# google/dynamic-video-depth

Hardware: AMD Instinct MI355X
Metric: train iters/s (depth+sceneflow step) at 384x672, 48 pairs; warp+loss HBM GB/s (higher is better)
Workload: dtype f32 (storage and accumulation fp32; conv / MLP contractions on v_mfma_f32_32x32x16_f16: every fp32 operand, scaled by a power of two from its tensor's max, is split into two fp16 terms (22 bits) and a product is three partial products; <= 4e-6 of max|y| against float64, the bound the 3-term bf16 / 6

## Files before the change

### dynamic-video-depth_amd/dvd_hip/csrc/xconv.hip

```cpp
#include <type_traits>

#include "dvd_split.h"
#include "xconv_tile.h"

namespace dvd {

typedef float f32x16 __attribute__((ext_vector_type(16)));
typedef float f32x2 __attribute__((ext_vector_type(2)));
typedef unsigned u32x4 __attribute__((ext_vector_type(4)));

#ifndef DVD_XCONV_ROLL
#define DVD_XCONV_ROLL 1
#endif
#ifndef DVD_XCONV_SPARE
#define DVD_XCONV_SPARE 0
#endif
#ifndef DVD_XCONV_DIRECT_BATCH
#define DVD_XCONV_DIRECT_BATCH 4
#endif
constexpr int kXHeader = 16;

__device__ __forceinline__ float xconv_weight(const float* __restrict__ w, int co_g, int idx, const float* __restrict__ sc_gamma,
                                              const float* __restrict__ sc_var, float sc_eps) {
  float val = w[idx];
// ... 134 lines not shown
      for (int k = 0; k < 4; ++k) m = fmaxf(fmaxf(m, fmaxf(fabsf(v[k].x), fabsf(v[k].y))), fmaxf(fabsf(v[k].z), fabsf(v[k].w)));
      if (it.var) m *= fabsf((it.gamma ? it.gamma[row] : 1.0f) / sqrtf(it.var[row] + it.eps));
      mall = fmaxf(mall, m);
    }
  } else {
    for (int row = blockIdx.x * kWamaxWaves + wave; row < it.rows; row += gridDim.x * kWamaxWaves) {
      const float* wr = it.w + (size_t)row * it.row_len;
      float m = 0.0f;
      for (int i = lane; i < it.row_len; i += 64) m = fmaxf(m, fabsf(wr[i]));
      if (it.var) m *= fabsf((it.gamma ? it.gamma[row] : 1.0f) / sqrtf(it.var[row] + it.eps));
      mall = fmaxf(mall, m);
    }
  }
  block_partial_max<kWamaxWaves>(mall, reinterpret_cast<float*>(it.packed));
}

__global__ __launch_bounds__(256) void xconv_pack_many_kernel(const XPackDev* __restrict__ table, int n) {
  int lo = 0, hi = n - 1;
  while (lo < hi) {
    const int mid = (lo + hi + 1) >> 1;
    if (table[mid].block0 <= blockIdx.x) lo = mid; else hi = mid - 1;
  }
  const XPackDev it = table[lo];
  xconv_pack_block(it.w, it.packed, it.co, it.ci, it.T, it.transposed, it.mtiles, it.nkc, it.G, it.gamma, it.var, it.eps,
                   kManyPartials, blockIdx.x - it.block0);
}

struct XArgs {
  const void* __restrict__ x;
  const uint4* __restrict__ wp;
  const float* __restrict__ bias;
  const void* __restrict__ res;
  const void* __restrict__ mask_src;
  const float* __restrict__ bn_gamma;
  const float* __restrict__ bn_beta;
  const float* __restrict__ bn_mean;
  const float* __restrict__ bn_var;
  float bn_eps;
  const float* __restrict__ x_amax;
  float* y_amax;
  void* __restrict__ y;
  int N, Cin, Cout, H, W;
  int G, mbpg, mtiles;
  int KS, pad, T;
  int TR, TC, P, ntr, ntc, NV;
  int PQ;
  int nkc, npos, nfi;
  int relu_in, relu_out, res_relu;
  int vec_out;
  int Hi, Wi, S2, ZI;
};

constexpr int kXFitOne = 11;
template <int TM, int TN, int WM, int WN, int FIT, bool FAST, bool B1 = false, bool IN16 = false, bool OUT16 = false>
__global__ __launch_bounds__(64 * WM * WN, B1 ? 3 : 2) void xconv_kernel(const XArgs a) {
  static_assert(!IN16 || FAST, "fp16 activations exist on the buffer-addressed main loop only");
  using TX = std::conditional_t<IN16, _Float16, float>;
  using TY = std::conditional_t<OUT16, _Float16, float>;
  using RawT = std::conditional_t<IN16, unsigned short, float>;
  constexpr int BT = IN16 ? 1 : 2;
  constexpr int XB = IN16 ? 2 : 4;
  constexpr int NT = 64 * WM * WN;
  constexpr bool kDirect = FIT == 0;
  constexpr bool kOne = FIT == kXFitOne;
  constexpr int FI = (kDirect || kOne) ? 1 : FIT;
  constexpr int MT = WM * TM;
  constexpr int AU = MT * 2 * 64;
  constexpr int AI = (AU + NT - 1) / NT;
  constexpr int AS = AI * NT;
  extern __shared__ __attribute__((aligned(16))) u32x4 smem[];
  u32x4* sA = smem;
  u32x4* sB = smem + 2 * AS;
  const int tid = threadIdx.x, lane = tid & 63, wave = tid >> 6;
  const int wm = wave / WN, wn = wave - wm * WN;
  const int tr = blockIdx.x / a.ntc, tc = blockIdx.x - tr * a.ntc;
  const int r0 = tr * a.TR, c0 = tc * a.TC;
  const int grp = blockIdx.y / a.mbpg;
  const int mt0 = (blockIdx.y - grp * a.mbpg) * MT;
  const int n = blockIdx.z;
  const size_t plane = (size_t)a.H * a.W;
  const size_t planeI = (size_t)a.Hi * a.Wi;
  const TX* xn = static_cast<const TX*>(a.x) + ((size_t)n * a.G + grp) * a.Cin * planeI;
  const int npos = a.npos, P = a.P, T = a.T, KS = a.KS;
  const int nkt = a.nkc * T;

  auto locate = [&](int p, bool live, int& go, bool& ok, int& lp) {
    if (a.S2) {
      const int PI = 2 * a.TC + 1;
      const int rr = p / PI, cc = p - rr * PI;
      const int row = 2 * r0 - 1 + rr, col = 2 * c0 - 1 + cc;
      ok = live && row >= 0 && row < a.Hi && col >= 0 && col < a.Wi;
      go = ok ? (row * a.Wi + col) : 0;
      lp = ((rr & 1) * 2 + (cc & 1)) * a.S2 + (rr >> 1) * P + (cc >> 1);
      return;
    }
    const int rr = p / P, cc = p - rr * P;
    const int row = r0 - a.pad + rr, col = c0 - a.pad + cc;
    ok = live && row >= 0 && row < a.H && col >= 0 && col < a.W;
    if (a.ZI) {
      ok = ok && !((row | col) & 1);
      go = ok ? ((row >> 1) * a.Wi + (col >> 1)) : 0;
    } else {
      go = ok ? (row * a.W + col) : 0;
    }
    lp = p;
  };
  auto tapoff = [&](int ky, int kx) { return xconv_tapoff(ky, kx, P, a.S2); };
  int goff[FI], lidx[FI], cig8[FI];
  bool gok[FI];
#pragma unroll
  for (int it = 0; it < FI; ++it) {
    const int item = it * NT + tid;
    const int cig = item >= a.NV ? 1 : 0;
    const int p = item - cig * a.NV;
    const bool live = item < 2 * a.NV;
    int lp;
    locate(p, live, goff[it], gok[it], lp);
    lidx[it] = live ? (cig * npos + lp) : (npos - 1);
    cig8[it] = live ? cig * 8 : 0;
  }
  const int planeB = (int)planeI * XB;
  const float sx = IN16 ? 1.0f : pow2_scale(a.x_amax[0]);
  const float sw = pow2_scale(reinterpret_cast<const float*>(a.wp)[0]);
  int voff[FI];
#pragma unroll
// ... 162 lines not shown
        }
      }
      uint4 h, l;
      split8_f16(v, sx, h, l);
      dst[li] = (u32x4){h.x, h.y, h.z, h.w};
      dst[2 * npos + li] = (u32x4){l.x, l.y, l.z, l.w};
    }
  };

  const u32x4* asrc[AI];
#pragma unroll
  for (int i = 0; i < AI; ++i) {
    const int j = i * NT + tid;
    const int jj = j < AU ? j : 0;
    const int mtl = jj / 128, rem = jj - mtl * 128;
    asrc[i] = reinterpret_cast<const u32x4*>(a.wp) + kXHeader + ((size_t)(grp * a.mtiles + mt0 + mtl) * nkt) * 128 + rem;
  }
  const u32x4* abase = reinterpret_cast<const u32x4*>(a.wp) + kXHeader + ((size_t)(grp * a.mtiles + mt0) * nkt) * 128;
  const __amdgpu_buffer_rsrc_t srdA = __builtin_amdgcn_make_buffer_rsrc(
      uniform_ptr(const_cast<u32x4*>(abase)), 0, FAST ? MT * nkt * 128 * 16 : 0, 0x00020000);
  int aoff[AI];
#pragma unroll
  for (int i = 0; i < AI; ++i) {
    const int j = i * NT + tid;
    const int jj = j < AU ? j : 0;
    const int mtl = jj / 128, rem = jj - mtl * 128;
    aoff[i] = (mtl * nkt * 128 + rem) * 16;
  }
  struct ARegs {
    u32x4 v[AI];
  };
  auto load_a = [&](ARegs& r, int kt) {
    if (FAST) {
#pragma unroll
      for (int i = 0; i < AI; ++i)
        r.v[i] = __builtin_bit_cast(u32x4, __builtin_amdgcn_raw_buffer_load_b128(srdA, aoff[i], kt * 2048, 0));
      return;
    }
#pragma unroll
    for (int i = 0; i < AI; ++i) r.v[i] = asrc[i][(size_t)kt * 128];
  };
  auto write_a = [&](const ARegs& r, int buf) {
#pragma unroll
    for (int i = 0; i < AI; ++i) sA[buf * AS + i * NT + tid] = r.v[i];
  };

  f32x16 acc[TM][TN];
#pragma unroll
  for (int tm = 0; tm < TM; ++tm)
#pragma unroll
    for (int tn = 0; tn < TN; ++tn) acc[tm][tn] = (f32x16){0, 0, 0, 0, 0, 0, 0, 0, 0, 0, 0, 0, 0, 0, 0, 0};

  auto qpos = [&](int tn) { return (wn * TN + tn) * 32 + (lane & 31); };
  constexpr bool kPackCells = TM >= 4 && !kOne;
  constexpr int QP = kPackCells ? (TN + 1) / 2 : TN;
  int qbp[QP];
#pragma unroll
  for (int h = 0; h < QP; ++h) {
    if constexpr (kPackCells) {
      const int c0 = xconv_cell(qpos(2 * h), a.PQ, P, a.TR);
      const int c1 = 2 * h + 1 >= TN ? 0 : xconv_cell(qpos(2 * h + 1), a.PQ, P, a.TR);
      qbp[h] = c0 | (c1 << 16);
    } else {
      qbp[h] = kOne ? 0 : xconv_cell(qpos(h), a.PQ, P, a.TR);
    }
  }
  auto cells = [&](int (&qb)[TN]) {
    if constexpr (kOne) {
#pragma unroll
      for (int tn = 0; tn < TN; ++tn) qb[tn] = qpos(tn);
    } else if constexpr (!kPackCells) {
#pragma unroll
      for (int tn = 0; tn < TN; ++tn) qb[tn] = qbp[tn];
    } else {
#pragma unroll
      for (int h = 0; h < QP; ++h) {
        int pk = qbp[h];
        asm volatile("" : "+v"(pk));
        qb[2 * h] = pk & 0xffff;
        if (2 * h + 1 < TN) qb[2 * h + 1] = (int)((unsigned)pk >> 16);
      }
    }
  };
  const int bl = (lane >> 5) * npos;
  const int al = (wm * TM) * 128 + lane;

  struct Frag {
    f16x8 a[TM][2], b[TN][BT];
  };
  auto read_frags = [&](Frag& f, int abuf, int kc, int off) {
    const u32x4* Ac = sA + abuf * AS + al;
    const u32x4* Bc = sB + (B1 ? 0 : (kc & 1) * 2 * BT * npos) + bl + off;
    int qb[TN];
    cells(qb);
#pragma unroll
    for (int tm = 0; tm < TM; ++tm)
#pragma unroll
      for (int s = 0; s < 2; ++s) f.a[tm][s] = __builtin_bit_cast(f16x8, Ac[(tm * 2 + s) * 64]);
#pragma unroll
    for (int tn = 0; tn < TN; ++tn)
#pragma unroll
      for (int s = 0; s < BT; ++s) f.b[tn][s] = __builtin_bit_cast(f16x8, Bc[s * 2 * npos + qb[tn]]);
  };
  auto mfmas = [&](const Frag& f) {
#define DVD_XTERM(SA, SB)                                                                             \
  _Pragma("unroll") for (int tm = 0; tm < TM; ++tm) _Pragma("unroll") for (int tn = 0; tn < TN; ++tn) \
      acc[tm][tn] = __builtin_amdgcn_mfma_f32_32x32x16_f16(f.a[tm][SA], f.b[tn][SB], acc[tm][tn], 0, 0, 0);
    DVD_XTERM(1, 0)
    if constexpr (!IN16) { DVD_XTERM(0, 1) }
    DVD_XTERM(0, 0)
#undef DVD_XTERM
  };

  constexpr bool kSingleA = TM >= 4;
  constexpr bool kRoll = kSingleA && !B1 && (DVD_XCONV_ROLL != 0);
  ARegs ra, rb;
  if (kRoll) {
    load_a(ra, 0);
    if (!kDirect) load_raw(0);
    write_a(ra, 0);
    load_a(ra, nkt > 1 ? 1 : 0);
    if (kDirect) {
      stage_direct(0, 0);
      if (T == 1 && a.nkc > 1) stage_direct(1, 1);
    } else {
      split_write(0, 0);
      load_raw(a.nkc > 1 ? 1 : 0);
      if (T == 1) {
        if (a.nkc > 1) split_write(1, 1);
        load_raw(a.nkc > 2 ? 2 : 0);
      }
    }
    write_a(ra, 1);
    __syncthreads();
    f16x8 fa[TM][2], fb[2][TN][BT];
    {
      const u32x4* Ac = sA + al;
      const u32x4* Bc = sB + bl;
      int qb[TN];
      cells(qb);
#pragma unroll
      for (int tm = 0; tm < TM; ++tm)
#pragma unroll
        for (int t = 0; t < 2; ++t) fa[tm][t] = __builtin_bit_cast(f16x8, Ac[(tm * 2 + t) * 64]);
#pragma unroll
      for (int tn = 0; tn < TN; ++tn)
#pragma unroll
        for (int t = 0; t < BT; ++t) fb[0][tn][t] = __builtin_bit_cast(f16x8, Bc[t * 2 * npos + qb[tn]]);
    }
    int nc = 0, ny = 0, nx = 0;
    auto advance = [&]() {
      if (++nx == KS) {
        nx = 0;
        if (++ny == KS) {
          ny = 0;
          ++nc;
        }
      }
    };
    advance();
    auto step_roll = [&](int kt, f16x8 (&bc)[TN][BT], f16x8 (&bn)[TN][BT]) {
      __syncthreads();
      load_a(ra, kt + 2 < nkt ? kt + 2 : kt);
      const u32x4* Ac = sA + ((kt + 1) & 1) * AS + al;
      const u32x4* Bc = sB + (nc & 1) * 2 * BT * npos + bl + tapoff(ny, nx);
      int qb[TN];
      cells(qb);
#pragma unroll
      for (int tn = 0; tn < TN; ++tn)
#pragma unroll
// ... 89 lines not shown
    split_write(0, 0);
    load_raw(a.nkc > 1 ? 1 : 0);
  }

  int kc = 0, ky = 0, kx = 0;
  auto step = [&](int kt, ARegs& rn) {
    __syncthreads();
    Frag f;
    read_frags(f, kt & 1, kc, tapoff(ky, kx));
    if (kSingleA) {
      load_a(rn, kt + 1 < nkt ? kt + 1 : kt);
      __builtin_amdgcn_sched_barrier(0);
    }
    mfmas(f);
    write_a(rn, (kt + 1) & 1);
    if (!kSingleA) load_a(rn, kt + 3 < nkt ? kt + 3 : kt);
    if (++kx == KS) {
      kx = 0;
      if (++ky == KS) {
        ky = 0;
        if (B1) __syncthreads();
        if (kDirect) {
          if (kc + 1 < a.nkc) stage_direct((kc + 1) & 1, kc + 1);
        } else {
#if DVD_XCONV_SPARE
          split_write((kc + 1) & 1, kc + 1);
          load_raw(kc + 2 < a.nkc ? kc + 2 : kc);
#else
          if (kc + 1 < a.nkc) split_write((kc + 1) & 1, kc + 1);
          if (kc + 2 < a.nkc) load_raw(kc + 2);
#endif
        }
        ++kc;
      }
    }
  };
  if (kSingleA) {
    for (int kt = 0; kt < nkt; ++kt) step(kt, ra);
  } else {
    for (int kt = 0; kt < nkt; kt += 2) {
      step(kt, rb);
      if (kt + 1 < nkt) step(kt + 1, ra);
    }
  }
  }

  const int TRv = (a.H - r0) < a.TR ? (a.H - r0) : a.TR;
  const int TCv = (a.W - c0) < a.TC ? (a.W - c0) : a.TC;
  const size_t ibase = ((size_t)n * a.G + grp) * a.Cout * plane;
  TY* __restrict__ yb = static_cast<TY*>(a.y) + ibase;
  const int iplane = (int)plane;
  const float unscale = 1.0f / (sx * sw);
  float ymax = 0.0f;
  if constexpr (kOne) {
    if (a.vec_out) {
      constexpr int PXL = OUT16 ? 8 : 4;
      constexpr int LPR = 64 / PXL;
      constexpr int RPI = 64 / LPR;
      constexpr int kTP = 68;
      __syncthreads();
      float* Tw = reinterpret_cast<float*>(smem) + wave * (32 * kTP);
      const int j = lane & 31, hh = lane >> 5;
      const int px = (lane % LPR) * PXL, rl = lane / LPR;
      const int q0 = wn * TN * 32;
      const bool pok = q0 + px < TCv;
      float my_sc[TM], my_sh[TM];
#pragma unroll
      for (int tm = 0; tm < TM; ++tm) {
        my_sc[tm] = 1.0f;
        my_sh[tm] = 0.0f;
        if (a.bn_var) {
          const int co = (mt0 + wm * TM + tm) * 32 + (lane & 31);
          const int cg = grp * a.Cout + (co < a.Cout ? co : a.Cout - 1);
          my_sc[tm] = (a.bn_gamma ? a.bn_gamma[cg] : 1.0f) / sqrtf(a.bn_var[cg] + a.bn_eps);
          my_sh[tm] = (a.bn_beta ? a.bn_beta[cg] : 0.0f) - a.bn_mean[cg] * my_sc[tm];
        }
      }
#pragma unroll
      for (int tm = 0; tm < TM; ++tm) {
#pragma unroll
        for (int tn = 0; tn < TN; ++tn)
#pragma unroll
          for (int r = 0; r < 16; ++r)
            Tw[((r & 3) + 8 * (r >> 2) + 4 * hh) * kTP + tn * 32 + j] = acc[tm][tn][r] * unscale;
        __builtin_amdgcn_wave_barrier();
#pragma unroll
        for (int i = 0; i < 32 / RPI; ++i) {
          const int cl = rl + RPI * i;
          const int co = (mt0 + wm * TM + tm) * 32 + cl;
          const bool ok = pok && co < a.Cout;
          float v[PXL];
#pragma unroll
          for (int e4 = 0; e4 < PXL; e4 += 4) {
            const float4 t = *reinterpret_cast<const float4*>(Tw + cl * kTP + px + e4);
            v[e4] = t.x; v[e4 + 1] = t.y; v[e4 + 2] = t.z; v[e4 + 3] = t.w;
          }
          const int cg = grp * a.Cout + (co < a.Cout ? co : a.Cout - 1);
          if (a.bias) {
            const float b = a.bias[cg];
#pragma unroll
            for (int e = 0; e < PXL; ++e) v[e] += b;
          }
          if (a.bn_var) {
            const float sc = __shfl(my_sc[tm], cl, 64), sh = __shfl(my_sh[tm], cl, 64);
#pragma unroll
            for (int e = 0; e < PXL; ++e) v[e] = __builtin_fmaf(v[e], sc, sh);
          }
          const int o = ok ? co * iplane + c0 + q0 + px : 0;
          auto load_run = [&](const void* base, float (&d)[PXL]) {
            const TY* __restrict__ p = static_cast<const TY*>(base) + ibase + o;
            if constexpr (OUT16) {
              const u32x4 t = *reinterpret_cast<const u32x4*>(p);
#pragma unroll
              for (int e = 0; e < 4; ++e) {
                const f16x2 h2 = __builtin_bit_cast(f16x2, (unsigned)t[e]);
                d[2 * e] = (float)h2[0];
                d[2 * e + 1] = (float)h2[1];
              }
            } else {
              const float4 t = *reinterpret_cast<const float4*>(p);
              d[0] = t.x; d[1] = t.y; d[2] = t.z; d[3] = t.w;
            }
          };
          if (a.res) {
            float rv[PXL];
            load_run(a.res, rv);
#pragma unroll
            for (int e = 0; e < PXL; ++e) v[e] += a.res_relu ? fmaxf(rv[e], 0.0f) : rv[e];
          }
          if (a.mask_src) {
            float mv[PXL];
            load_run(a.mask_src, mv);
#pragma unroll
            for (int e = 0; e < PXL; ++e) v[e] = mv[e] > 0.0f ? v[e] : 0.0f;
          }
          if (a.relu_out) {
#pragma unroll
// ... 53 lines not shown
          const int co = cob + (r & 3) + 8 * (r >> 2);
          v[r] += a.bias[grp * a.Cout + (co < a.Cout ? co : a.Cout - 1)];
        }
      }
      if (a.bn_var) {
#pragma unroll
        for (int r = 0; r < 16; ++r) {
          const int src = (r & 3) + 8 * (r >> 2) + 4 * (lane >> 5);
          v[r] = __builtin_fmaf(v[r], __shfl(my_sc[tm], src, 64), __shfl(my_sh[tm], src, 64));
        }
      }
      if (a.res) {
        const TY* __restrict__ rb = static_cast<const TY*>(a.res) + ibase;
        float rv[16];
#pragma unroll
        for (int r = 0; r < 16; ++r) {
          const int co = cob + (r & 3) + 8 * (r >> 2);
          rv[r] = (float)rb[(full || co < a.Cout) ? o0 + ((r & 3) + 8 * (r >> 2)) * iplane : pix];
        }
#pragma unroll
        for (int r = 0; r < 16; ++r) v[r] += a.res_relu ? fmaxf(rv[r], 0.0f) : rv[r];
      }
      if (a.mask_src) {
        const TY* __restrict__ mb = static_cast<const TY*>(a.mask_src) + ibase;
        float mv[16];
#pragma unroll
        for (int r = 0; r < 16; ++r) {
          const int co = cob + (r & 3) + 8 * (r >> 2);
          mv[r] = (float)mb[(full || co < a.Cout) ? o0 + ((r & 3) + 8 * (r >> 2)) * iplane : pix];
        }
#pragma unroll
        for (int r = 0; r < 16; ++r) v[r] = mv[r] > 0.0f ? v[r] : 0.0f;
      }
      if (a.relu_out) {
#pragma unroll
        for (int r = 0; r < 16; ++r) v[r] = fmaxf(v[r], 0.0f);
      }
#pragma unroll
      for (int r = 0; r < 16; ++r) {
        const int co = cob + (r & 3) + 8 * (r >> 2);
        if (pok && (full || co < a.Cout)) {
          yb[o0 + ((r & 3) + 8 * (r >> 2)) * iplane] = (TY)v[r];
          ymax = amax_acc(ymax, v[r]);
        }
      }
    }
  }
  if (a.y_amax) wave_amax_to(ymax, a.y_amax);
}

static int g_xcfg = 0;

template <int TM, int TN, int WM, int WN, bool FAST, bool B1 = false, bool IN16 = false, bool OUT16 = false>
static int launch_fi(const XArgs& a, int FI, dim3 grid, size_t lds, hipStream_t s) {
  auto go = [&](auto kern) -> int {
    DVD_HIP_OK(hipFuncSetAttribute(reinterpret_cast<const void*>(kern), hipFuncAttributeMaxDynamicSharedMemorySize, (int)lds));
    hipLaunchKernelGGL(kern, grid, dim3(64 * WM * WN), lds, s, a);
    DVD_LAUNCH_OK();
    return DVD_OK;
  };
  const double flops = 2.0 * a.N * (double)a.G * a.Cout * a.Cin * a.T * (double)a.H * a.W * (a.ZI ? 0.25 : 1.0);
  if constexpr (TM >= 4 && !B1 && FAST && DVD_XCONV_ROLL != 0) {
    if (a.T == 1 && FI == 1 && g_xcfg != 6) {
      flops_add(DVD_FLOP_XCONV_1X1_WIDE, flops);
      return go(xconv_kernel<TM, TN, WM, WN, kXFitOne, FAST, B1, IN16, OUT16>);
    }
  }
  flops_add(TM >= 4 ? DVD_FLOP_XCONV_WIDE : (WM == 2 ? DVD_FLOP_XCONV_128 : DVD_FLOP_XCONV_SMALL), flops);
  switch (FI) {
    case 1: return go(xconv_kernel<TM, TN, WM, WN, 1, FAST, B1, IN16, OUT16>);
    case 2: return go(xconv_kernel<TM, TN, WM, WN, 2, FAST, B1, IN16, OUT16>);
    case 3: return go(xconv_kernel<TM, TN, WM, WN, 3, FAST, B1, IN16, OUT16>);
    default: return go(xconv_kernel<TM, TN, WM, WN, 0, FAST, B1, IN16, OUT16>);
  }
}

static int xconv_mtiles(int M) {
  const int bm = M <= 32 ? 32 : (M <= 64 ? 64 : (M >= 256 ? 256 : 128));
  return (M + bm - 1) / bm * (bm / 32);
}

}

extern "C" {

size_t dvd_xconv_packed_bytes(int Cout, int Cin, int KS, int groups, int transposed) {
  if (Cout <= 0 || Cin <= 0 || KS <= 0 || !(KS & 1) || groups <= 0 || Cout % groups || Cin % groups) return 0;
  const int co = Cout / groups, ci = Cin / groups;
  const int M = transposed ? ci : co, K = transposed ? co : ci;
  return ((size_t)dvd::kXHeader + (size_t)groups * dvd::xconv_mtiles(M) * ((K + 15) / 16) * KS * KS * 2 * 64) * sizeof(uint4);
}

static int xconv_pack_impl(const float* w, void* packed, int Cout, int Cin, int KS, int groups, int transposed,
                           const float* gamma, const float* var, float eps, dvd_stream_t stream) {
  DVD_REQUIRE(w && packed, "xconv_pack: null pointer");
  DVD_REQUIRE(Cout > 0 && Cin > 0 && KS > 0 && (KS & 1) && KS <= 11 && groups > 0 && Cout % groups == 0 && Cin % groups == 0,
              "xconv_pack: bad shape Cout=%d Cin=%d KS=%d groups=%d", Cout, Cin, KS, groups);
  const int co = Cout / groups, ci = Cin / groups;
  const int M = transposed ? ci : co, K = transposed ? co : ci;
  const int mtiles = dvd::xconv_mtiles(M), nkc = (K + 15) / 16, T = KS * KS;
  const long long total = (long long)groups * mtiles * nkc * T * 64;
  dvd::bytes_add(DVD_BYTES_PACK, 8.0 * (double)Cout * ci * T + 16.0 * (double)total);
  const int row_len = ci * T;
  int npart;
  if (row_len % 4 == 0 && reinterpret_cast<uintptr_t>(w) % 16 == 0) {
    const int cpr = (row_len + 1023) / 1024;
    const long long nb = ((long long)Cout * cpr + dvd::kWamaxWaves - 1) / dvd::kWamaxWaves;
    npart = (int)(nb < dvd::kXPartials ? nb : dvd::kXPartials);
    hipLaunchKernelGGL(dvd::xconv_wamax4_kernel, dim3((unsigned)npart), dim3(64 * dvd::kWamaxWaves), 0, static_cast<hipStream_t>(stream), w,
                       static_cast<float*>(packed), Cout, row_len, cpr, gamma, var, eps);
    DVD_LAUNCH_OK();
  } else {
    npart = Cout < dvd::kXPartials ? Cout : dvd::kXPartials;
    hipLaunchKernelGGL(dvd::xconv_wamax_kernel, dim3((unsigned)npart), dim3(256), 0, static_cast<hipStream_t>(stream), w,
                       static_cast<float*>(packed), Cout, row_len, gamma, var, eps);
    DVD_LAUNCH_OK();
  }
  hipLaunchKernelGGL(dvd::xconv_pack_kernel, dim3((unsigned)((total + 255) / 256)), dim3(256), 0,
                     static_cast<hipStream_t>(stream), w, static_cast<uint4*>(packed), co, ci, T, transposed ? 1 : 0,
                     mtiles, nkc, groups, gamma, var, eps, npart);
  DVD_LAUNCH_OK();
  return DVD_OK;
}

int dvd_xconv_pack(const float* w, void* packed, int Cout, int Cin, int KS, int groups, int transposed, dvd_stream_t stream) {
  return xconv_pack_impl(w, packed, Cout, Cin, KS, groups, transposed, nullptr, nullptr, 0.0f, stream);
// ... 9 lines not shown

int dvd_xconv_pack_many(const dvd_xpack_item* items, int n, void* table, size_t table_bytes, int upload, dvd_stream_t stream) {
  DVD_REQUIRE(items && table && n > 0, "xconv_pack_many: bad arguments");
  DVD_REQUIRE(table_bytes >= dvd_xconv_pack_table_bytes(n), "xconv_pack_many: table %zu < %zu bytes", table_bytes,
              dvd_xconv_pack_table_bytes(n));
  std::vector<dvd::XPackDev> host((size_t)n);
  unsigned long long blocks = 0;
  double bytes = 0.0;
  for (int i = 0; i < n; ++i) {
    const dvd_xpack_item& q = items[i];
    DVD_REQUIRE(q.w && q.packed, "xconv_pack_many: item %d: null pointer", i);
    DVD_REQUIRE(q.Cout > 0 && q.Cin > 0 && q.KS > 0 && (q.KS & 1) && q.KS <= 11 && q.groups > 0 && q.Cout % q.groups == 0 &&
                    q.Cin % q.groups == 0,
                "xconv_pack_many: item %d: bad shape Cout=%d Cin=%d KS=%d groups=%d", i, q.Cout, q.Cin, q.KS, q.groups);
    DVD_REQUIRE(!q.gamma || q.var, "xconv_pack_many: item %d: BatchNorm scale without a variance", i);
    dvd::XPackDev& d = host[(size_t)i];
    d.w = q.w;
    d.packed = static_cast<uint4*>(q.packed);
    d.gamma = q.gamma;
    d.var = q.var;
    d.eps = q.eps;
    d.co = q.Cout / q.groups;
    d.ci = q.Cin / q.groups;
    d.T = q.KS * q.KS;
    d.transposed = q.transposed ? 1 : 0;
    const int M = d.transposed ? d.ci : d.co, K = d.transposed ? d.co : d.ci;
    d.mtiles = dvd::xconv_mtiles(M);
    d.nkc = (K + 15) / 16;
    d.G = q.groups;
    d.rows = q.Cout;
    d.row_len = d.ci * d.T;
    d.block0 = (unsigned)blocks;
    d.pad_ = 0;
    const long long total = (long long)d.G * d.mtiles * d.nkc * d.T * 64;
    blocks += (unsigned long long)((total + 255) / 256);
    bytes += 8.0 * (double)q.Cout * d.ci * d.T + 16.0 * (double)total;
  }
  DVD_REQUIRE(blocks < (1ull << 31), "xconv_pack_many: too many blocks");
  hipStream_t st = static_cast<hipStream_t>(stream);
  if (upload) {
    DVD_HIP_OK(hipMemcpyAsync(table, host.data(), (size_t)n * sizeof(dvd::XPackDev), hipMemcpyHostToDevice, st));
    DVD_HIP_OK(hipStreamSynchronize(st));
  }
  dvd::bytes_add(DVD_BYTES_PACK, bytes);
  const dvd::XPackDev* t = static_cast<const dvd::XPackDev*>(table);
  hipLaunchKernelGGL(dvd::xconv_wamax_many_kernel, dim3(dvd::kManyPartials, (unsigned)n), dim3(64 * dvd::kWamaxWaves), 0, st, t);
  DVD_LAUNCH_OK();
  hipLaunchKernelGGL(dvd::xconv_pack_many_kernel, dim3((unsigned)blocks), dim3(256), 0, st, t, n);
  DVD_LAUNCH_OK();
  return DVD_OK;
}

int dvd_xconv_select(int cfg) {
  DVD_REQUIRE(cfg >= 0 && cfg <= dvd::kXSelHalo, "xconv_select: cfg %d", cfg);
  dvd::g_xcfg = cfg;
  return DVD_OK;
}

static int xconv_fwd_impl(const void* x, const float* x_amax, const void* packed, const float* bias, const void* residual,
                          const void* mask_src, const dvd_bn_params* bn, void* y, float* y_amax, int N, int Cin_total,
                          int Cout_total, int H, int W, int KS, int groups, int flags, int in16, int out16, dvd_stream_t stream) {
  DVD_REQUIRE(x && packed && y, "xconv: null pointer");
  DVD_REQUIRE(in16 || x_amax, "xconv: the input's max|x| scalar is missing (dvd_amax, or the producer's y_amax)");
  DVD_REQUIRE(N > 0 && Cin_total > 0 && Cout_total > 0 && H > 0 && W > 0, "xconv: bad shape N=%d Cin=%d Cout=%d H=%d W=%d", N,
              Cin_total, Cout_total, H, W);
  DVD_REQUIRE(groups > 0 && Cin_total % groups == 0 && Cout_total % groups == 0, "xconv: %d groups do not divide the channels",
              groups);
  DVD_REQUIRE(KS > 0 && (KS & 1) && KS <= 11, "xconv: kernel size %d (odd sizes up to 11)", KS);
  DVD_REQUIRE(N <= 65535, "xconv: too many images for the grid");
  DVD_REQUIRE((long long)H * W * (long long)(Cin_total > Cout_total ? Cin_total : Cout_total) < (1ll << 31),
              "xconv: image too large for 32-bit offsets");
  DVD_REQUIRE(in16 || !out16, "xconv: fp32 input with fp16 output is not a configuration of this kernel");
  const int s2 = (flags >> 3) & 1, zi = (flags >> 4) & 1;
  DVD_REQUIRE(!(s2 && zi), "xconv: stride-2 forward and stride-2 backward-data are different launches");
  DVD_REQUIRE(!(s2 || zi) || KS == 3, "xconv: the strided forms exist for 3x3 kernels (got %d)", KS);
  const int Hq = (H + 1) / 2, Wq = (W + 1) / 2;
  const int Cin = Cin_total / groups, Cout = Cout_total / groups;
  dvd::XPlan plan;
  const bool planned = dvd::xconv_plan(Cin, Cout, H, W, KS, s2 != 0, in16 != 0, dvd::g_xcfg, plan);
  const bool fast = plan.fast;
  DVD_REQUIRE(fast || !in16, "xconv: fp16 activations need input channels in multiples of 16 (got %d per group)", Cin);
  DVD_REQUIRE(!(s2 || zi) || fast, "xconv: the strided forms need input channels in multiples of 16 (got %d per group)", Cin);
  DVD_REQUIRE(planned, "xconv: no %stile of a %dx%d image with a %dx%d kernel fits the LDS", s2 ? "stride-2 " : "", H, W, KS, KS);
  const dvd::XCfg& c = plan.c;
  const dvd::XTile& t = plan.t;
  const int Hh = plan.Hh, Ww = plan.Ww, S2 = plan.S2;
  dvd::XArgs a;
  a.x = x;
  a.wp = static_cast<const uint4*>(packed);
  a.bias = bias;
  a.res = residual;
  a.mask_src = mask_src;
  a.bn_gamma = bn ? bn->gamma : nullptr;
  a.bn_beta = bn ? bn->beta : nullptr;
  a.bn_mean = bn ? bn->mean : nullptr;
  a.bn_var = bn ? bn->var : nullptr;
  a.bn_eps = bn ? bn->eps : 0.0f;
  DVD_REQUIRE(!bn || (bn->mean && bn->var), "xconv: BatchNorm statistics missing");
  a.y = y;
  a.x_amax = x_amax;
  a.y_amax = y_amax;
  a.N = N; a.Cin = Cin; a.Cout = Cout; a.H = Hh; a.W = Ww;
  a.G = groups; a.mtiles = dvd::xconv_mtiles(Cout);
  a.KS = KS; a.pad = KS / 2; a.T = KS * KS;
  a.TR = t.TR; a.TC = t.TC; a.P = t.P; a.PQ = t.PQ; a.ntr = t.ntr; a.ntc = t.ntc; a.NV = t.NV;
  a.nkc = (Cin + 15) / 16; a.npos = t.npos; a.nfi = t.FI;
  a.Hi = s2 ? H : (zi ? Hq : Hh); a.Wi = s2 ? W : (zi ? Wq : Ww); a.S2 = S2; a.ZI = zi;
  a.relu_in = flags & 1; a.relu_out = (flags >> 1) & 1; a.res_relu = (flags >> 2) & 1;
  const int mblocks = plan.mblocks;
  a.mbpg = mblocks;
  DVD_REQUIRE((long long)mblocks * groups <= 65535, "xconv: too many channel blocks");
  const dim3 grid(t.ntr * t.ntc, mblocks * groups, N);
  auto al16 = [](const void* p) { return (reinterpret_cast<uintptr_t>(p) & 15) == 0; };
  a.vec_out = (KS == 1 && ((long long)H * W) % 8 == 0 && t.TC % 8 == 0 && al16(y) && al16(residual) && al16(mask_src) &&
               dvd::g_xcfg != 7) ? 1 : 0;
  size_t lds = t.lds;
  if (a.vec_out && lds < (size_t)c.NT() / 64 * 32 * 68 * 4) lds = (size_t)c.NT() / 64 * 32 * 68 * 4;
  hipStream_t s = static_cast<hipStream_t>(stream);
#define DVD_XGO(TM_, TN_, WM_, WN_)                                                                                      \
  do {                                                                                                                   \
    if (in16 && out16) return dvd::launch_fi<TM_, TN_, WM_, WN_, true, false, true, true>(a, t.FI, grid, lds, s);         \
    if (in16) return dvd::launch_fi<TM_, TN_, WM_, WN_, true, false, true, false>(a, t.FI, grid, lds, s);                 \
    return dvd::launch_fi<TM_, TN_, WM_, WN_, true>(a, t.FI, grid, lds, s);                                               \
  } while (0)
  if (fast) {
    if (c.TM == 4 && c.WN == 4) DVD_XGO(4, 2, 2, 4);
    if (c.TM == 4) DVD_XGO(4, 2, 2, 2);
    if (c.WM == 2 && c.b1) return dvd::launch_fi<2, 2, 2, 2, true, true>(a, t.FI, grid, lds, s);
    if (c.TM == 2 && c.WM == 1 && c.b1) return dvd::launch_fi<2, 2, 1, 4, true, true>(a, t.FI, grid, lds, s);
    if (c.TM == 1 && c.b1) return dvd::launch_fi<1, 2, 1, 4, true, true>(a, t.FI, grid, lds, s);
    if (c.WM == 2) DVD_XGO(2, 2, 2, 2);
    if (c.TM == 2) DVD_XGO(2, 2, 1, 4);
    DVD_XGO(1, 2, 1, 4);
  }
#undef DVD_XGO
  if (c.WM == 2) return dvd::launch_fi<2, 2, 2, 2, false>(a, t.FI, grid, lds, s);
  if (c.TM == 2) return dvd::launch_fi<2, 2, 1, 4, false>(a, t.FI, grid, lds, s);
  return dvd::launch_fi<1, 2, 1, 4, false>(a, t.FI, grid, lds, s);
}

int dvd_xconv_fwd(const float* x, const float* x_amax, const void* packed, const float* bias, const float* residual,
                  const float* mask_src, const dvd_bn_params* bn, float* y, float* y_amax, int N, int Cin_total, int Cout_total,
                  int H, int W, int KS, int groups, int flags, dvd_stream_t stream) {
  return xconv_fwd_impl(x, x_amax, packed, bias, residual, mask_src, bn, y, y_amax, N, Cin_total, Cout_total, H, W, KS, groups,
                        flags, 0, 0, stream);
}

int dvd_xconv_fwd_h(const void* x, const void* packed, const float* bias, const void* residual, const void* mask_src,
                    const dvd_bn_params* bn, void* y, float* y_amax, int N, int Cin_total, int Cout_total, int H, int W, int KS,
                    int groups, int flags, int out_f16, dvd_stream_t stream) {
  return xconv_fwd_impl(x, nullptr, packed, bias, residual, mask_src, bn, y, y_amax, N, Cin_total, Cout_total, H, W, KS, groups,
                        flags, 1, out_f16 ? 1 : 0, stream);
}

}
```

### dynamic-video-depth_amd/dvd_hip/csrc/xconv_tile.h

```cpp
#pragma once
#include <cstddef>

#if defined(__HIPCC__) || defined(__CUDACC__)
#define DVD_XTILE_HD __host__ __device__
#else
#define DVD_XTILE_HD
#endif

namespace dvd {

DVD_XTILE_HD inline int xconv_cell(int q, int PQ, int P, int TR) {
  const int rr = q / PQ;
  return rr < TR ? rr * P + (q - rr * PQ) : 0;
}
DVD_XTILE_HD inline int xconv_tapoff(int ky, int kx, int P, int S2) {
  return S2 ? ((ky & 1) * 2 + (kx & 1)) * S2 + (ky >> 1) * P + (kx >> 1) : ky * P + kx;
}

struct XCfg {
  int TM, TN, WM, WN;
  bool b1 = false;
  bool in16 = false;
  int blockM() const { return TM * WM * 32; }
  int NQ() const { return TN * WN * 32; }
  int NT() const { return 64 * WM * WN; }
};
constexpr int kXSelHalo = 8;
inline XCfg pick_cfg(int M, int KS, int sel) {
  if (M <= 32) return {1, 2, 1, 4};
  if (M <= 64) return {2, 2, 1, 4};
  if (M > 64 && sel == 5) return {2, 2, 2, 2, true};
  if (M >= 256 && sel != 1 && sel != 4) {
    if (sel == 2) return {4, 2, 2, 2};
    if (sel == 3) return {4, 2, 2, 4};
    return KS == 1 ? XCfg{4, 2, 2, 2} : XCfg{4, 2, 2, 4};
  }
  return {2, 2, 2, 2};
}
constexpr int kXLdsBudget = 78 * 1024;
constexpr int kXLdsBudgetOne = 156 * 1024;
constexpr int kXLdsBudgetB1 = 52 * 1024;
constexpr int kXMaxFI = 3;
constexpr int kXMaxFIDirect = 16;

struct XTile {
  int TR, TC, P, PQ, ntr, ntc, NV, npos, FI;
  size_t lds;
};
inline size_t xconv_lds(const XCfg& c, int npos) {
  const int AU = c.WM * c.TM * 128, NT = c.NT();
  const int AS = (AU + NT - 1) / NT * NT;
  return ((size_t)2 * AS + (size_t)(c.b1 ? 4 : 8) * npos / (c.in16 ? 2 : 1)) * 16;
}
inline bool pick_tile_halo_budget(int H, int W, int KS, const XCfg& c, XTile& best, int budget) {
  const int pad = KS / 2, NQ = c.NQ(), NT = c.NT();
  double best_eff = -1.0;
  for (int nct = 1; nct <= W; ++nct) {
    int TC = (W + nct - 1) / nct;
    if (KS == 1) TC = (TC + 7) & ~7;
    const int P = TC + 2 * pad;
    if (P > NQ) continue;
    const int ntc = (W + TC - 1) / TC;
    const int npos = NQ + (KS - 1) * (P + 1) + 1;
    if (xconv_lds(c, npos) > (size_t)budget) continue;
    int trmax = NQ / P;
    if (trmax > H) trmax = H;
    for (int tr0 = trmax; tr0 >= 1; --tr0) {
      const int ntr = (H + tr0 - 1) / tr0;
      const int TR = (H + ntr - 1) / ntr;
      const int NV = (TR + 2 * pad) * P;
      const int FI = (2 * NV + NT - 1) / NT;
      if (FI > kXMaxFIDirect) continue;
      const double eff = (double)H * W / ((double)ntr * ntc * NQ) - 0.02 * (double)NV / (TR * TC) - 1e-6 * nct;
      if (eff > best_eff) {
        best_eff = eff;
        best = {TR, TC, P, P, ntr, ntc, NV, npos, FI, xconv_lds(c, npos)};
      }
      break;
    }
    if (TC <= 8) break;
  }
  return best_eff > -1.0;
}
constexpr double kXWideSlack = 0.02;
constexpr int kXWideTC = 32;
inline bool pick_tile_dense_budget(int H, int W, int KS, const XCfg& c, XTile& best, int budget, int fi_min, int fi_max) {
  const int pad = KS / 2, NQ = c.NQ(), NT = c.NT();
  double best_eff = -1.0, wide_eff = -1.0;
  XTile wide{};
  for (int nct = 1; nct <= W; ++nct) {
    const int TC = (W + nct - 1) / nct;
    if (TC > NQ) continue;
    const int P = TC + 2 * pad;
    const int ntc = (W + TC - 1) / TC;
    int trmax = NQ / TC;
    if (trmax > H) trmax = H;
    for (int tr0 = trmax; tr0 >= 1; --tr0) {
      const int ntr = (H + tr0 - 1) / tr0;
      const int TR = (H + ntr - 1) / ntr;
      const int NV = (TR + 2 * pad) * P;
      const int npos = NV + 1;
      const int FI = (2 * NV + NT - 1) / NT;
// ... 61 lines not shown
    if (xconv_lds(c, npos) <= (size_t)budget && FI <= 4 * kXMaxFIDirect) {
      const double eff = (double)Ho * Wo / ((double)ntr * ntc * NQ) - 1e-6 * nct;
      if (eff > best_eff) {
        best_eff = eff;
        best = {TR, TC, P, PQ, ntr, ntc, NV, npos, FI, xconv_lds(c, npos)};
        S2 = s2;
      }
    }
    if (TC <= 4) break;
  }
  return best_eff > -1.0;
}
inline bool pick_tile_s2(int Ho, int Wo, const XCfg& c, XTile& best, int& S2, bool halo) {
  const int budgets[2] = {kXLdsBudget, kXLdsBudgetOne};
  for (int budget : budgets) {
    XTile h;
    int sh = 0;
    if (!pick_tile_s2_budget(Ho, Wo, c, h, sh, budget, true)) continue;
    best = h;
    S2 = sh;
    if (halo) return true;
    XTile d;
    int sd = 0;
    const int tier = h.lds <= (size_t)kXLdsBudgetB1 ? kXLdsBudgetB1 : budget;
    if (pick_tile_s2_budget(Ho, Wo, c, d, sd, tier, false) && d.ntr * d.ntc <= h.ntr * h.ntc) {
      best = d;
      S2 = sd;
    } else {
      best.PQ = h.TC;
      best.npos = 3 * sh + h.TR * h.P + 1;
      best.lds = xconv_lds(c, best.npos);
    }
    return true;
  }
  return false;
}

struct XPlan {
  XCfg c;
  XTile t;
  int S2;
  int Hh, Ww;
  bool fast;
  int mblocks;
};
inline bool xconv_plan(int Cin, int Cout, int H, int W, int KS, bool s2, bool in16, int sel, XPlan& p) {
  p.fast = (Cin % 16 == 0) && ((long long)Cin * H * W * 4 < (1ll << 31)) &&
           ((long long)8 * ((Cin + 15) / 16) * KS * KS * 2048 < (1ll << 31)) && sel != 4;
  p.c = pick_cfg((p.fast && !s2) ? Cout : (Cout < 128 ? Cout : 128), KS, sel);
  if (!p.fast) p.c.b1 = false;
  if (s2) p.c.b1 = true;
  if (in16) p.c.b1 = false;
  p.c.in16 = in16;
  p.Hh = H;
  p.Ww = W;
  if (KS == 1) {
    p.Hh = 1;
    p.Ww = H * W;
  }
  p.S2 = 0;
  const bool halo = sel == kXSelHalo || xconv_keeps_halo_positions(Cin, Cout, H, W, KS, s2);
  bool ok;
  if (s2) {
    p.Hh = (H + 1) / 2;
    p.Ww = (W + 1) / 2;
    ok = pick_tile_s2(p.Hh, p.Ww, p.c, p.t, p.S2, halo);
  } else {
    if (p.c.b1 && !pick_tile(p.Hh, p.Ww, KS, p.c, p.t, halo)) p.c.b1 = false;
    ok = pick_tile(p.Hh, p.Ww, KS, p.c, p.t, halo);
  }
  p.mblocks = (Cout + p.c.blockM() - 1) / p.c.blockM();
  return ok;
}

}
```

### dynamic-video-depth_amd/dvd_hip/ops.py

```python
import ctypes
import os
import sys

import torch

from . import _lib

CAM_KEYS = ('R_1', 'R_2', 'R_1_T', 'R_2_T', 't_1', 't_2', 'K', 'K_inv')


def _p(t):
    return ctypes.c_void_p(t.data_ptr()) if t is not None else ctypes.c_void_p(0)


def _stream():
    return ctypes.c_void_p(torch.cuda.current_stream().cuda_stream)


def _dev32(t, name):
    if not (torch.is_tensor(t) and t.is_cuda):
        raise RuntimeError('%s must be a GPU tensor (dvd_hip has no CPU path)' % name)
    if t.dtype != torch.float32:
        raise RuntimeError('%s must be float32, got %s' % (name, t.dtype))
    return t if t.is_contiguous() else t.contiguous()
# ... 653 lines not shown
    return am


_ws_cache = {}


def _workspace(nbytes, device):
    if torch.cuda.is_current_stream_capturing():
        return torch.empty(max(nbytes, 1 << 20), device=device, dtype=torch.uint8)
    key = (device.index, torch.cuda.current_stream().cuda_stream)
    ws = _ws_cache.get(key)
    if ws is None or ws.numel() < nbytes:
        ws = torch.empty(max(nbytes, 1 << 20), device=device, dtype=torch.uint8)
        _ws_cache[key] = ws
    return ws


def warp_loss_fused(cfg, depth_1, depth_2, flow_1_2, mask_2, sf_1_2, cams, grads=True, out=None):
    depth_1, depth_2 = _dev32(depth_1, 'depth_1'), _dev32(depth_2, 'depth_2')
    flow_1_2, mask_2, sf_1_2 = _dev32(flow_1_2, 'flow_1_2'), _dev32(mask_2, 'mask_2'), _dev32(sf_1_2, 'sf_1_2')
    B, H, W = cfg.B, cfg.H, cfg.W
    if depth_1.numel() != B * H * W or depth_2.numel() != B * H * W or mask_2.numel() != B * H * W:
        raise RuntimeError('warp_loss_fused: depth/mask shape does not match cfg %dx%dx%d' % (B, H, W))
    if flow_1_2.numel() != 2 * B * H * W or sf_1_2.numel() != 3 * B * H * W:
        raise RuntimeError('warp_loss_fused: flow / scene-flow shape mismatch')
    cst, keep = pack_cameras(cams)
    dev = depth_1.device
    lib = _lib.load()
    nws = lib.dvd_warp_loss_workspace_bytes(B, H, W)
    ws = _workspace(nws, dev)
    if out is not None:
        sums, g1, g2, gs = out
    else:
        sums = torch.empty(4, device=dev, dtype=torch.float32)
        g1 = torch.empty_like(depth_1) if grads else None
        g2 = torch.empty_like(depth_2) if grads else None
        gs = torch.empty_like(sf_1_2) if grads else None
    if grads:
        st = lib.dvd_warp_loss_fused(ctypes.byref(cfg), _p(depth_1), _p(depth_2), _p(flow_1_2), _p(mask_2),
                                     _p(sf_1_2), ctypes.byref(cst), _p(ws), ws.numel(), _p(sums), _p(g1), _p(g2),
                                     _p(gs), _stream())
        _lib.check(st, 'dvd_warp_loss_fused')
    else:
        st = lib.dvd_warp_loss_fwd(ctypes.byref(cfg), _p(depth_1), _p(depth_2), _p(flow_1_2), _p(mask_2),
                                   _p(sf_1_2), ctypes.byref(cst), _p(ws), ws.numel(), _p(sums), _stream())
        _lib.check(st, 'dvd_warp_loss_fwd')
    del keep
    return sums, g1, g2, gs


FLOP_CLASSES = ('xconv_1x1_wide', 'xconv_wide', 'xconv_128', 'xconv_small', 'xwgrad3', 'xwgrad3g', 'xwgrad1b', 'xwgrad1s',
                'xwgradk', 'mlp_fwd', 'mlp_bwd_dx', 'mlp_bwd_dw')
FLOP_CLASS_KERNELS = {
    'xconv_1x1_wide': ('xconv_kernelILi4ELi2ELi2ELi2ELi11E', 'xconv_kernel<4, 2, 2, 2, 11,'),
    'xconv_wide': ('xconv_kernelILi4ELi2ELi2ELi4E', 'xconv_kernelILi4ELi2ELi2ELi2ELi0E', 'xconv_kernelILi4ELi2ELi2ELi2ELi1E',
                   'xconv_kernelILi4ELi2ELi2ELi2ELi2E', 'xconv_kernelILi4ELi2ELi2ELi2ELi3E', 'xconv_kernel<4, 2, 2, 4,',
                   'xconv_kernel<4, 2, 2, 2, 0,', 'xconv_kernel<4, 2, 2, 2, 1,', 'xconv_kernel<4, 2, 2, 2, 2,',
                   'xconv_kernel<4, 2, 2, 2, 3,'),
    'xconv_128': ('xconv_kernelILi2ELi2ELi2ELi2E', 'xconv_kernel<2, 2, 2, 2,'),
    'xconv_small': ('xconv_kernelILi1ELi2ELi1ELi4E', 'xconv_kernelILi2ELi2ELi1ELi4E', 'xconv_kernel<1, 2, 1, 4,',
                    'xconv_kernel<2, 2, 1, 4,'),
    'xwgrad3': ('xwgrad3_kernel',), 'xwgrad3g': ('xwgrad3g_kernel',), 'xwgrad1b': ('xwgrad1b_kernel',),
    'xwgrad1s': ('xwgrad1s_kernel',), 'xwgradk': ('xwgradk_kernel',),
    'mlp_fwd': ('mlp_fwd_kernel',), 'mlp_bwd_dx': ('mlp_bwd_dx_kernel',), 'mlp_bwd_dw': ('mlp_bwd_dw_kernel',),
}


BYTE_CLASSES = ('bnrelu_fwd', 'bnrelu_bwd', 'upsample_fwd', 'upsample_bwd', 'amax', 'pack', 'pool', 'gconv_c8', 'elementwise',
                'adam', 'geometry', 'gather')
BYTE_CLASS_KERNELS = {
    'bnrelu_fwd': ('bnrelu_fwd_kernel',), 'bnrelu_bwd': ('bnrelu_bwd', 'bn_mask', 'bnrelu_sum'),
    'upsample_fwd': ('upsample_bilinear_fwd', 'bicubic_fwd_kernel'),
    'upsample_bwd': ('upsample_bilinear_bwd', 'upsample_bwd', 'bicubic_bwd_'),
    'amax': ('amax_kernel', 'chansum_'), 'pack': ('xconv_wamax', 'xconv_pack_kernel'), 'pool': ('maxpool3s2', 'subsample2_', 'avgpool_'),
    'gconv_c8': ('gconv3x3_c8',), 'elementwise': ('mul_mask_kernel', 'scale_add_kernel', 'acc_reg_kernel', 'sum_partials_kernel',
                                                  'head1x1_', 'cast_scale_kernel'),
    'adam': ('adam_kernel', 'sgd_kernel'), 'geometry': ('unproject_', 'track_project_kernel', 'project_bwd_kernel', 'splat_zmin_kernel', 'splat_accumulate_kernel',
                                                   'splat_resolve_kernel', 'eval_tracks_kernel', 'ratio_hist_kernel', 'ratio_pick_kernel',
                                                   'depth_score_kernel'), 'gather': ('gather_pairs_kernel', 'store_gather_kernel', 'union_'),
}
ALL_CLASSES = FLOP_CLASSES + BYTE_CLASSES


def flop_counters(reset=False):
    lib = _lib.load()
    buf = (ctypes.c_double * len(FLOP_CLASSES))()
    _lib.check(lib.dvd_flop_counters(ctypes.cast(buf, ctypes.c_void_p), len(FLOP_CLASSES), 1 if reset else 0), 'dvd_flop_counters')
    out = dict(zip(FLOP_CLASSES, [float(v) for v in buf]))
    bbuf = (ctypes.c_double * len(BYTE_CLASSES))()
    _lib.check(lib.dvd_byte_counters(ctypes.cast(bbuf, ctypes.c_void_p), len(BYTE_CLASSES), 1 if reset else 0), 'dvd_byte_counters')
    out.update(zip(BYTE_CLASSES, [float(v) for v in bbuf]))
    return out


REPLAYED = {k: 0.0 for k in ALL_CLASSES}


RECOMPUTED = {k: 0.0 for k in ALL_CLASSES}


class counting_recomputed(object):

    def __enter__(self):
        self.before = executed_flops()
        return self

    def __exit__(self, *exc):
# ... 490 lines not shown
```

Baseline: 1.676.

## Add 1x1 conv kernel streaming weight fragments from L2 instead of LDS

Adds a new 1x1 xconv variant (FIT=12, 2x4 tiles with 4x1 waves) that loads A/weight fragments straight into registers with buffer loads, double-buffered across K steps. LDS then holds only the split activation tiles in a 4-slot ring. The intent is to cut LDS traffic and shared-memory footprint for wide 1x1 convolutions and overlap global loads with MFMA work. By default it replaces the TM=4, WN=2 1x1 config, and the old path stays reachable through a new select value. The epilogue is reworked to write tiles in pairs. The cost is more register pressure and reliance on L2 hits for weights.

New measurement: 1.692 (median of 6 runs). About the same (+0.9%).

```diff
diff --git a/dynamic-video-depth_amd/dvd_hip/csrc/xconv.hip b/dynamic-video-depth_amd/dvd_hip/csrc/xconv.hip
--- a/dynamic-video-depth_amd/dvd_hip/csrc/xconv.hip
+++ b/dynamic-video-depth_amd/dvd_hip/csrc/xconv.hip
@@ -210,6 +210,7 @@
 };
 
 constexpr int kXFitOne = 11;
+constexpr int kXFitOneL2 = 12;
 template <int TM, int TN, int WM, int WN, int FIT, bool FAST, bool B1 = false, bool IN16 = false, bool OUT16 = false>
 __global__ __launch_bounds__(64 * WM * WN, B1 ? 3 : 2) void xconv_kernel(const XArgs a) {
   static_assert(!IN16 || FAST, "fp16 activations exist on the buffer-addressed main loop only");
@@ -221,14 +222,17 @@
   constexpr int NT = 64 * WM * WN;
   constexpr bool kDirect = FIT == 0;
   constexpr bool kOne = FIT == kXFitOne;
-  constexpr int FI = (kDirect || kOne) ? 1 : FIT;
+  constexpr bool kOneL2 = FIT == kXFitOneL2;
+  static_assert(!kOneL2 || (FAST && !B1 && !IN16 && TN % 2 == 0), "the L2-weights 1x1 loop: buffer loads, fp32 storage");
+  constexpr bool kOneAny = kOne || kOneL2;
+  constexpr int FI = (kDirect || kOneAny) ? 1 : FIT;
   constexpr int MT = WM * TM;
   constexpr int AU = MT * 2 * 64;
   constexpr int AI = (AU + NT - 1) / NT;
   constexpr int AS = AI * NT;
   extern __shared__ __attribute__((aligned(16))) u32x4 smem[];
   u32x4* sA = smem;
-  u32x4* sB = smem + 2 * AS;
+  u32x4* sB = smem + (kOneL2 ? 0 : 2 * AS);
   const int tid = threadIdx.x, lane = tid & 63, wave = tid >> 6;
   const int wm = wave / WN, wn = wave - wm * WN;
   const int tr = blockIdx.x / a.ntc, tc = blockIdx.x - tr * a.ntc;
@@ -497,7 +501,7 @@
     for (int tn = 0; tn < TN; ++tn) acc[tm][tn] = (f32x16){0, 0, 0, 0, 0, 0, 0, 0, 0, 0, 0, 0, 0, 0, 0, 0};
 
   auto qpos = [&](int tn) { return (wn * TN + tn) * 32 + (lane & 31); };
-  constexpr bool kPackCells = TM >= 4 && !kOne;
+  constexpr bool kPackCells = TM >= 4 && !kOneAny;
   constexpr int QP = kPackCells ? (TN + 1) / 2 : TN;
   int qbp[QP];
 #pragma unroll
@@ -507,11 +511,11 @@
       const int c1 = 2 * h + 1 >= TN ? 0 : xconv_cell(qpos(2 * h + 1), a.PQ, P, a.TR);
       qbp[h] = c0 | (c1 << 16);
     } else {
-      qbp[h] = kOne ? 0 : xconv_cell(qpos(h), a.PQ, P, a.TR);
+      qbp[h] = kOneAny ? 0 : xconv_cell(qpos(h), a.PQ, P, a.TR);
     }
   }
   auto cells = [&](int (&qb)[TN]) {
-    if constexpr (kOne) {
+    if constexpr (kOneAny) {
 #pragma unroll
       for (int tn = 0; tn < TN; ++tn) qb[tn] = qpos(tn);
     } else if constexpr (!kPackCells) {
@@ -560,7 +564,72 @@
   constexpr bool kSingleA = TM >= 4;
   constexpr bool kRoll = kSingleA && !B1 && (DVD_XCONV_ROLL != 0);
   ARegs ra, rb;
-  if (kRoll) {
+  if constexpr (kOneL2) {
+    static_assert(kXOneG == 2, "the loop below is written for two K steps per stage");
+    const int arow = __builtin_amdgcn_readfirstlane(wm * TM) * nkt * 2048;
+    const int avo = lane * 16;
+    f16x8 fa[2][TM][2], fb[TN][BT];
+    auto req_a = [&](f16x8 (&f)[TM][2], int kt) {
+#pragma unroll
+      for (int tm = 0; tm < TM; ++tm)
+#pragma unroll
+        for (int t = 0; t < 2; ++t)
+          f[tm][t] = __builtin_bit_cast(
+              f16x8, __builtin_amdgcn_raw_buffer_load_b128(srdA, avo + t * 1024, arow + (tm * nkt + kt) * 2048, 0));
+    };
+    auto chunk = [&](int c) { return c < a.nkc ? c : a.nkc - 1; };
+    const u32x4* Bl = sB + bl + wn * TN * 32 + (lane & 31);
+    auto read_b = [&](int tn, int buf) {
+#pragma unroll
+      for (int t = 0; t < BT; ++t)
+        fb[tn][t] = __builtin_bit_cast(f16x8, Bl[(buf * 2 * BT + t * 2) * npos + tn * 32]);
+    };
+    auto sub = [&](const f16x8 (&ac)[TM][2], int nbuf) {
+#pragma unroll
+      for (int tn = 0; tn < TN; ++tn) {
+#pragma unroll
+        for (int tm = 0; tm < TM; ++tm)
+          acc[tm][tn] = __builtin_amdgcn_mfma_f32_32x32x16_f16(ac[tm][1], fb[tn][0], acc[tm][tn], 0, 0, 0);
+#pragma unroll
+        for (int tm = 0; tm < TM; ++tm)
+          acc[tm][tn] = __builtin_amdgcn_mfma_f32_32x32x16_f16(ac[tm][0], fb[tn][1], acc[tm][tn], 0, 0, 0);
+#pragma unroll
+        for (int tm = 0; tm < TM; ++tm)
+          acc[tm][tn] = __builtin_amdgcn_mfma_f32_32x32x16_f16(ac[tm][0], fb[tn][0], acc[tm][tn], 0, 0, 0);
+        __builtin_amdgcn_sched_barrier(0);
+        read_b(tn, nbuf);
+        __builtin_amdgcn_sched_barrier(0);
+      }
+    };
+    req_a(fa[0], 0);
+    load_raw_to(raw, 0);
+    load_raw_to(raw_b, chunk(1));
+    split_write_from(raw, 0, 0);
+    split_write_from(raw_b, 1, 1);
+    load_raw_to(raw, chunk(2));
+    load_raw_to(raw_b, chunk(3));
+    split_write_from(raw, 2, 2);
+    split_write_from(raw_b, 3, 3);
+    __syncthreads();
+#pragma unroll
+    for (int tn = 0; tn < TN; ++tn) read_b(tn, 0);
+    for (int k0 = 0; k0 < nkt; k0 += 2) {
+      const int st = (k0 >> 1) & 1;
+      req_a(fa[1], k0 + 1 < nkt ? k0 + 1 : k0);
+      load_raw_to(raw, chunk(k0 + 4));
+      load_raw_to(raw_b, chunk(k0 + 5));
+      __builtin_amdgcn_sched_barrier(0);
+      sub(fa[0], st * 2 + 1);
+      if (k0 + 1 < nkt) {
+        __syncthreads();
+        req_a(fa[0], k0 + 2 < nkt ? k0 + 2 : k0);
+        __builtin_amdgcn_sched_barrier(0);
+        sub(fa[1], (st ^ 1) * 2);
+        split_write_from(raw, st * 2, k0 + 4);
+        split_write_from(raw_b, st * 2 + 1, k0 + 5);
+      }
+    }
+  } else if (kRoll) {
     load_a(ra, 0);
     if (!kDirect) load_raw(0);
     write_a(ra, 0);
@@ -756,7 +825,7 @@
   const int iplane = (int)plane;
   const float unscale = 1.0f / (sx * sw);
   float ymax = 0.0f;
-  if constexpr (kOne) {
+  if constexpr (kOneAny) {
     if (a.vec_out) {
       constexpr int PXL = OUT16 ? 8 : 4;
       constexpr int LPR = 64 / PXL;
@@ -766,8 +835,7 @@
       float* Tw = reinterpret_cast<float*>(smem) + wave * (32 * kTP);
       const int j = lane & 31, hh = lane >> 5;
       const int px = (lane % LPR) * PXL, rl = lane / LPR;
-      const int q0 = wn * TN * 32;
-      const bool pok = q0 + px < TCv;
+      constexpr int NH = TN / 2;
       float my_sc[TM], my_sh[TM];
 #pragma unroll
       for (int tm = 0; tm < TM; ++tm) {
@@ -781,12 +849,15 @@
         }
       }
 #pragma unroll
-      for (int tm = 0; tm < TM; ++tm) {
-#pragma unroll
-        for (int tn = 0; tn < TN; ++tn)
+      for (int th = 0; th < TM * NH; ++th) {
+        const int tm = th / NH, hf = th - tm * NH;
+        const int q0 = (wn * TN + 2 * hf) * 32;
+        const bool pok = q0 + px < TCv;
+#pragma unroll
+        for (int tn = 0; tn < 2; ++tn)
 #pragma unroll
           for (int r = 0; r < 16; ++r)
-            Tw[((r & 3) + 8 * (r >> 2) + 4 * hh) * kTP + tn * 32 + j] = acc[tm][tn][r] * unscale;
+            Tw[((r & 3) + 8 * (r >> 2) + 4 * hh) * kTP + tn * 32 + j] = acc[tm][2 * hf + tn][r] * unscale;
         __builtin_amdgcn_wave_barrier();
 #pragma unroll
         for (int i = 0; i < 32 / RPI; ++i) {
@@ -946,7 +1017,7 @@
 static int g_xcfg = 0;
 
 template <int TM, int TN, int WM, int WN, bool FAST, bool B1 = false, bool IN16 = false, bool OUT16 = false>
-static int launch_fi(const XArgs& a, int FI, dim3 grid, size_t lds, hipStream_t s) {
+static int launch_fi(const XArgs& a, int FI, dim3 grid, size_t lds, hipStream_t s, bool l2a = false) {
   auto go = [&](auto kern) -> int {
     DVD_HIP_OK(hipFuncSetAttribute(reinterpret_cast<const void*>(kern), hipFuncAttributeMaxDynamicSharedMemorySize, (int)lds));
     hipLaunchKernelGGL(kern, grid, dim3(64 * WM * WN), lds, s, a);
@@ -954,6 +1025,11 @@
     return DVD_OK;
   };
   const double flops = 2.0 * a.N * (double)a.G * a.Cout * a.Cin * a.T * (double)a.H * a.W * (a.ZI ? 0.25 : 1.0);
+  if constexpr (TM == 2 && TN == 4 && WM == 4 && WN == 1 && FAST && !B1 && !IN16) {
+    DVD_REQUIRE(l2a && a.T == 1 && FI == 1, "xconv: the L2-weights 1x1 kernel got T=%d FI=%d", a.T, FI);
+    flops_add(DVD_FLOP_XCONV_1X1_WIDE, flops);
+    return go(xconv_kernel<TM, TN, WM, WN, kXFitOneL2, FAST, B1, IN16, OUT16>);
+  } else {
   if constexpr (TM >= 4 && !B1 && FAST && DVD_XCONV_ROLL != 0) {
     if (a.T == 1 && FI == 1 && g_xcfg != 6) {
       flops_add(DVD_FLOP_XCONV_1X1_WIDE, flops);
@@ -966,6 +1042,7 @@
     case 2: return go(xconv_kernel<TM, TN, WM, WN, 2, FAST, B1, IN16, OUT16>);
     case 3: return go(xconv_kernel<TM, TN, WM, WN, 3, FAST, B1, IN16, OUT16>);
     default: return go(xconv_kernel<TM, TN, WM, WN, 0, FAST, B1, IN16, OUT16>);
+  }
   }
 }
 
@@ -1081,7 +1158,7 @@
 }
 
 int dvd_xconv_select(int cfg) {
-  DVD_REQUIRE(cfg >= 0 && cfg <= dvd::kXSelHalo, "xconv_select: cfg %d", cfg);
+  DVD_REQUIRE(cfg >= 0 && cfg <= dvd::kXSelMax, "xconv_select: cfg %d", cfg);
   dvd::g_xcfg = cfg;
   return DVD_OK;
 }
@@ -1153,6 +1230,7 @@
     return dvd::launch_fi<TM_, TN_, WM_, WN_, true>(a, t.FI, grid, lds, s);                                               \
   } while (0)
   if (fast) {
+    if (c.l2a) return dvd::launch_fi<2, 4, 4, 1, true>(a, t.FI, grid, lds, s, true);
     if (c.TM == 4 && c.WN == 4) DVD_XGO(4, 2, 2, 4);
     if (c.TM == 4) DVD_XGO(4, 2, 2, 2);
     if (c.WM == 2 && c.b1) return dvd::launch_fi<2, 2, 2, 2, true, true>(a, t.FI, grid, lds, s);
diff --git a/dynamic-video-depth_amd/dvd_hip/csrc/xconv_tile.h b/dynamic-video-depth_amd/dvd_hip/csrc/xconv_tile.h
--- a/dynamic-video-depth_amd/dvd_hip/csrc/xconv_tile.h
+++ b/dynamic-video-depth_amd/dvd_hip/csrc/xconv_tile.h
@@ -21,11 +21,15 @@
   int TM, TN, WM, WN;
   bool b1 = false;
   bool in16 = false;
+  bool l2a = false;
   int blockM() const { return TM * WM * 32; }
   int NQ() const { return TN * WN * 32; }
   int NT() const { return 64 * WM * WN; }
 };
 constexpr int kXSelHalo = 8;
+constexpr int kXSelOneLds = 9;
+constexpr int kXSelMax = 9;
+constexpr int kXOneG = 2;
 inline XCfg pick_cfg(int M, int KS, int sel) {
   if (M <= 32) return {1, 2, 1, 4};
   if (M <= 64) return {2, 2, 1, 4};
@@ -48,6 +52,7 @@
   size_t lds;
 };
 inline size_t xconv_lds(const XCfg& c, int npos) {
+  if (c.l2a) return (size_t)2 * kXOneG * 4 * npos * 16;
   const int AU = c.WM * c.TM * 128, NT = c.NT();
   const int AS = (AU + NT - 1) / NT * NT;
   return ((size_t)2 * AS + (size_t)(c.b1 ? 4 : 8) * npos / (c.in16 ? 2 : 1)) * 16;
@@ -215,6 +220,10 @@
   if (s2) p.c.b1 = true;
   if (in16) p.c.b1 = false;
   p.c.in16 = in16;
+  if (KS == 1 && p.c.TM == 4 && p.c.WN == 2 && !in16 && sel != 6 && sel != kXSelOneLds) {
+    p.c = XCfg{2, 4, 4, 1};
+    p.c.l2a = true;
+  }
   p.Hh = H;
   p.Ww = W;
   if (KS == 1) {
diff --git a/dynamic-video-depth_amd/dvd_hip/ops.py b/dynamic-video-depth_amd/dvd_hip/ops.py
--- a/dynamic-video-depth_amd/dvd_hip/ops.py
+++ b/dynamic-video-depth_amd/dvd_hip/ops.py
@@ -729,7 +729,8 @@
 FLOP_CLASSES = ('xconv_1x1_wide', 'xconv_wide', 'xconv_128', 'xconv_small', 'xwgrad3', 'xwgrad3g', 'xwgrad1b', 'xwgrad1s',
                 'xwgradk', 'mlp_fwd', 'mlp_bwd_dx', 'mlp_bwd_dw')
 FLOP_CLASS_KERNELS = {
-    'xconv_1x1_wide': ('xconv_kernelILi4ELi2ELi2ELi2ELi11E', 'xconv_kernel<4, 2, 2, 2, 11,'),
+    'xconv_1x1_wide': ('xconv_kernelILi4ELi2ELi2ELi2ELi11E', 'xconv_kernel<4, 2, 2, 2, 11,',
+                       'xconv_kernelILi2ELi4ELi4ELi1ELi12E', 'xconv_kernel<2, 4, 4, 1, 12,'),
     'xconv_wide': ('xconv_kernelILi4ELi2ELi2ELi4E', 'xconv_kernelILi4ELi2ELi2ELi2ELi0E', 'xconv_kernelILi4ELi2ELi2ELi2ELi1E',
                    'xconv_kernelILi4ELi2ELi2ELi2ELi2E', 'xconv_kernelILi4ELi2ELi2ELi2ELi3E', 'xconv_kernel<4, 2, 2, 4,',
                    'xconv_kernel<4, 2, 2, 2, 0,', 'xconv_kernel<4, 2, 2, 2, 1,', 'xconv_kernel<4, 2, 2, 2, 2,',
```
